# ofsouzap/DistributedMandelbrot

Measured on AMD Instinct MI355X. Metric: G pixel-iterations/s on 4096^2 tile, max_iter=1000 fp64, higher is better.
Workload: dtype f64

## Files before the change

distributedmandelbrot_amd/_lib.py:

```python
from __future__ import annotations

import ctypes as C
import importlib.util
import os
import sys

HERE = os.path.dirname(os.path.abspath(__file__))
SO_PATH = os.path.join(HERE, "libmbk_hip.so")

MBK_OK, MBK_ERR_INVALID, MBK_ERR_NO_DEVICE, MBK_ERR_HIP, MBK_ERR_NOMEM, MBK_ERR_NET = range(6)
MBK_WANT_COUNTS = 0x1
MBK_WANT_BYTES = 0x2
MBK_KERNEL_DEFAULT = 0x000
MBK_KERNEL_SIMPLE = 0x100
MBK_KERNEL_ASM = 0x200
MBK_KERNEL_REFILL = 0x300
MBK_KERNEL_GROUP = 0x400
MBK_KERNEL_SCAN = 0x500
KERNELS = {"default": MBK_KERNEL_DEFAULT, "simple": MBK_KERNEL_SIMPLE, "asm": MBK_KERNEL_ASM,
           "refill": MBK_KERNEL_REFILL, "group": MBK_KERNEL_GROUP, "scan": MBK_KERNEL_SCAN}
OPTIONS = {name: i for i, name in enumerate(
    ["order", "waves_per_wg", "group_steps", "exact_steps", "probe_steps", "scan_waves", "scan_xcd_map", "scan_col_period", "heavy_share",
     "rf_livemin", "rf_patience", "rf_batch", "rf_waves", "cycle_detect", "probe_mid", "prepass_overlap", "exact_long", "scan_inline", "wave_limit", "units_min_light", "xcd_balance", "m_late", "h_settled", "classify_wg", "scan_strip", "cycle_window", "spill_first", "spill_lanes", "spill_min_mrd", "spill_min_blocks", "spill_cyc_shift"])}
MBK_PRECISION_F32 = 0x1000
MBK_LAZY_UNIFORM = 0x2000
MBK_DEEP_BLA = 0x8000
MBK_DEEP_XBLA = 0x10000
PRECISIONS = {"f64": 0, "f32": MBK_PRECISION_F32}
MBK_SLOTS = 4
MBK_WORKER_DEPTH = 3
MBK_INFO_SCAN_WG_PER_CU = 100
MBK_INFO_XCD_SHARE = 110
MBK_INFO_SPILL = 130
MBK_CODEC_RAW = 0x00
MBK_CODEC_RLE = 0x01
MBK_CHUNK_DEFINITION = 4096
MBK_CHUNK_BYTES = 4096 * 4096
MBK_ABI_VERSION = 5
# ... 137 lines not shown
    "mbk_distance_value_host": (C.c_double, [C.c_double, C.c_double, C.c_int32]),
    "mbk_datachunk_submit": (C.c_int, [C.c_void_p, C.c_int, C.c_uint32, C.c_uint32, C.c_uint32, C.c_uint32,
                                       C.c_void_p, C.c_void_p]),
    "mbk_datachunk_submit_ex": (C.c_int, [C.c_void_p, C.c_int, C.c_uint32, C.c_uint32, C.c_uint32, C.c_uint32,
                                          C.c_void_p, C.c_void_p, C.c_uint32]),
    "mbk_view_submit": (C.c_int, [C.c_void_p, C.c_int, C.POINTER(mbk_view), C.c_uint32, C.c_uint32,
                                  C.c_void_p, C.c_void_p]),
    "mbk_wait": (C.c_int, [C.c_void_p, C.c_int, C.POINTER(mbk_stats)]),
    "mbk_serialize_last": (C.c_int, [C.c_void_p, C.c_void_p, C.c_uint64, C.POINTER(C.c_uint64),
                                     C.POINTER(C.c_uint32)]),
    "mbk_set_option": (C.c_int, [C.c_void_p, C.c_int, C.c_uint32]),
    "mbk_get_option": (C.c_int, [C.c_void_p, C.c_int, C.POINTER(C.c_uint32)]),
    "mbk_quantise_counts": (C.c_int, [C.c_void_p, C.c_void_p, C.c_uint64, C.c_uint32, C.c_void_p]),
    "mbk_units_plan": (C.c_int, [C.c_uint32, C.c_uint32, C.c_uint32, C.c_void_p, C.c_void_p]),
    "mbk_units_lookup": (C.c_int, [C.c_void_p, C.c_uint32, C.c_void_p, C.c_void_p]),
    "mbk_reduce_counts": (C.c_int, [C.c_void_p, C.c_void_p, C.c_uint64, C.c_uint32, C.c_void_p,
                                    C.POINTER(mbk_stats)]),
    "mbk_worker_run": (C.c_int, [C.c_void_p, C.c_char_p, C.c_uint16, C.c_uint64, C.c_uint32,
                                 C.POINTER(mbk_worker_report)]),
    "mbk_net_set_option": (C.c_int, [C.c_int, C.c_uint32]),
    "mbk_net_get_option": (C.c_int, [C.c_int, C.POINTER(C.c_uint32)]),
    "mbk_feeder_run": (C.c_int, [C.POINTER(mbk_feeder_ops), C.c_char_p, C.c_uint16, C.c_uint64, C.c_uint32,
                                 C.POINTER(mbk_worker_report)]),
    "mbk_deep_orbit_create": (C.c_int, [C.c_char_p, C.c_char_p, C.c_uint32, C.c_uint32, C.POINTER(C.c_void_p)]),
    "mbk_deep_orbit_destroy": (None, [C.c_void_p]),
    "mbk_deep_orbit_info": (C.c_int, [C.c_void_p, C.POINTER(C.c_uint32), C.POINTER(C.c_uint32), C.POINTER(C.c_uint32),
                                      C.POINTER(C.c_uint32)]),
    "mbk_deep_orbit_read": (C.c_int, [C.c_void_p, C.c_void_p, C.c_void_p, C.c_uint64]),
    "mbk_deep_view_launch": (C.c_int, [C.c_void_p, C.c_void_p, C.POINTER(mbk_deep_view), C.c_uint32, C.c_uint32,
                                       C.c_void_p, C.c_void_p, C.c_void_p, C.c_void_p]),
# ... 193 lines not shown
```

distributedmandelbrot_amd/csrc/mbk_api.hip:

```cpp
#include "../../include/mbk.h"

#include <hip/hip_runtime.h>

#include <cmath>
#include <cstdio>
#include <cstdlib>
#include <algorithm>
#include <cstring>
#include <new>
#include <string>
#include <vector>

#include "mbk_kernels.h"
#include "mbk_refill.h"
#include "mbk_persist.h"
#include "mbk_scan.h"
#include "mbk_units.h"
#include "mbk_spill.h"
#include "mbk_feeder.h"
#include "mbk_deep_orbit.h"
#include "mbk_deep.h"
#include "mbk_deep_bla.h"
#include "mbk_deep_wide.h"
#include "mbk_deep_wide_bla.h"
// ... 1042 lines not shown
    if (wb && mrd == 0) return fail(ctx, MBK_ERR_INVALID, "mrd == 0 has no quantised form (division by zero)");

    TileArgs a;
    std::memset(&a, 0, sizeof(a));
    fill_window(a, v);
    a.out_pitch = v->ncols;
    a.out_col0 = 0;
    a.out_row0 = 0;
    a.mrd = (int32_t)mrd;
    a.quant_wide = (mrd >= (1u << 23)) ? 1u : 0u;
    a.quant_rcp = mrd ? 1.0 / (double)mrd : 0.0;
    a.perm_mul = 1u;
    a.exact_steps = ctx->opt[MBK_OPT_EXACT_STEPS];
    a.exact_steps_long = std::min(ctx->opt[MBK_OPT_EXACT_STEPS], ctx->opt[MBK_OPT_EXACT_LONG]);
    a.cyc_window = ctx->opt[MBK_OPT_CYCLE_WINDOW];
    a.order = nullptr;
    a.counts = wc ? d_counts : nullptr;
    a.bytes = wb ? d_bytes : nullptr;
    a.smooth = d_smooth;

    const uint32_t kernel = flags & MBK_KERNEL_MASK;
    if (d_smooth && (f32 || kernel == MBK_KERNEL_SIMPLE || kernel == MBK_KERNEL_REFILL))
        return fail(ctx, MBK_ERR_INVALID, "smooth colouring is implemented by the fp64 scan / asm / group kernels only");
    if (f32 && (kernel == MBK_KERNEL_SIMPLE || kernel == MBK_KERNEL_REFILL))
        return fail(ctx, MBK_ERR_INVALID, "MBK_PRECISION_F32 is implemented by the scan / asm / group kernels only");
    switch (kernel) {
        case MBK_KERNEL_DEFAULT:
        case MBK_KERNEL_SCAN: {
            if (kernel == MBK_KERNEL_DEFAULT && (uint64_t)((a.ncols + 7u) / 8u) * ((a.nrows + 7u) / 8u) < 16384u)
                return launch_blocks(ctx, a, MBK_KERNEL_GROUP, safe, f32, stream);
// ... 415 lines not shown
    hipError_t e = hipGetDeviceCount(&n);
    if (e != hipSuccess || n <= 0)
        return fail(nullptr, MBK_ERR_NO_DEVICE,
                    std::string("no HIP device visible (") + hipGetErrorString(e) +
                        "); libmbk_hip has no CPU fallback");
    if (device < 0 || device >= n) return fail(nullptr, MBK_ERR_NO_DEVICE, "device index out of range");
    mbk_ctx *ctx = new (std::nothrow) mbk_ctx();
    if (!ctx) return fail(nullptr, MBK_ERR_NOMEM, "out of host memory");
    ctx->device = device;
    static const uint32_t kDefaults[MBK_OPT_COUNT_] = {
         3u,  1u,  16u,  8u,  32u,
         8u,  1u,  4u,  655u,
         48u,  256u,  1u,  8u,  1u,
         65537u,  1u,  0u,  1u,  0u,
         32768u,  0u,  8u,  6u,  1024u,
         1u,  32u,  256u,  16u,  2048u,  19u,  5u};
    std::memcpy(ctx->opt, kDefaults, sizeof(kDefaults));
#define MBK_CREATE_HIP(call)                                                        \
    do {                                                                            \
        hipError_t e2_ = (call);                                                    \
        if (e2_ != hipSuccess) {                                                    \
            fail(nullptr, MBK_ERR_HIP, std::string(#call) + ": " + hipGetErrorString(e2_)); \
            mbk_destroy(ctx);                                                       \
            return MBK_ERR_HIP;                                                     \
        }                                                                           \
    } while (0)
    MBK_CREATE_HIP(hipSetDevice(device));
    MBK_CREATE_HIP(hipGetDeviceProperties(&ctx->prop, device));
    if (std::strncmp(ctx->prop.gcnArchName, "gfx950", 6) != 0) {
        fail(nullptr, MBK_ERR_NO_DEVICE,
             std::string("device is ") + ctx->prop.gcnArchName + ", this library is built for gfx950 only");
// ... 604 lines not shown
        case MBK_OPT_CLASSIFY_WG: ok = value >= 64u && value <= 1024u && value % 64u == 0u; break;
        case MBK_OPT_SCAN_STRIP: ok = value <= 1u; break;
        case MBK_OPT_CYCLE_WINDOW: ok = value <= 65536u; break;
        case MBK_OPT_EXACT_LONG: ok = value <= 4096u; break;
        case MBK_OPT_SCAN_INLINE: ok = value <= 1u; break;
        case MBK_OPT_WAVE_LIMIT: ok = value <= 7u; break;
        case MBK_OPT_UNITS_MIN_LIGHT: ok = value <= 65536u; break;
        case MBK_OPT_XCD_BALANCE: ok = value <= 2u; break;
        case MBK_OPT_M_LATE: ok = value <= 65536u; break;
        case MBK_OPT_H_SETTLED: ok = value <= 30u; break;
        case MBK_OPT_SPILL_FIRST: ok = value <= 65536u && value % 32u == 0u; break;
        case MBK_OPT_SPILL_LANES: ok = value >= 1u && value <= 32u; break;
        case MBK_OPT_SPILL_MIN_MRD: ok = true; break;
        case MBK_OPT_SPILL_MIN_BLOCKS: ok = value <= 31u; break;
        case MBK_OPT_SPILL_CYC_SHIFT: ok = value <= 31u; break;
        default: return fail(ctx, MBK_ERR_INVALID, "unknown MBK_OPT_* selector");
    }
    if (!ok) return fail(ctx, MBK_ERR_INVALID, "option value out of range");
    ctx->opt[option] = value;
    return MBK_OK;
}

int mbk_get_option(mbk_ctx *ctx, int option, uint32_t *value)
{
    if (!ctx || !value) return fail(ctx, MBK_ERR_INVALID, "NULL argument");
    if (option >= MBK_INFO_SCAN_WG_PER_CU && option < MBK_INFO_SCAN_WG_PER_CU + 4) {
        const int k = option - MBK_INFO_SCAN_WG_PER_CU;
        *value = (uint32_t)ctx->scan_occ[k >> 1][k & 1];
        return MBK_OK;
    }
// ... 30 lines not shown
    double c = 0.0;
    for (uint32_t x = 0; x < 8u; ++x) {
        c += f[x];
        cum[x] = x == 7u ? (1u << 24) : (uint32_t)std::lround(std::min(1.0, std::max(0.0, c)) * (double)(1u << 24));
    }
}

int mbk_units_plan(uint32_t n_h, uint32_t n_v, uint32_t n_m, const double *fractions, uint32_t *plan)
{
    if (!fractions || !plan) return MBK_ERR_INVALID;
    if ((uint64_t)n_h + n_v + n_m > 0x7fffffffull) return MBK_ERR_INVALID;
    uint32_t cum[8];
    shares_from_fractions(fractions, cum);
    mbk::units_plan(n_h, n_v, n_m, cum, 0u, plan, 0u, 0u);
    return MBK_OK;
}

int mbk_units_lookup(const uint32_t *plan, uint32_t id, uint32_t *list, uint32_t *index)
{
    if (!plan || !list || !index) return MBK_ERR_INVALID;
    const uint32_t x = id & 7u;
    bool is_h = false;
    uint32_t i = 0;
    *list = 0u;
    *index = 0u;
    if (id >= plan[2] || !mbk::units_lookup(id, plan[3], plan[4], plan[8u + x], plan[16u + x], plan[24u + x], plan[32u + x], is_h, i))
        return MBK_OK;
    *list = is_h ? 1u : (i < plan[1] ? 2u : 3u);
    *index = is_h ? i : (i < plan[1] ? i : i - plan[1]);
    return MBK_OK;
// ... 2275 lines not shown
```

distributedmandelbrot_amd/csrc/mbk_kernels.h:

```cpp
#pragma once

#include <hip/hip_runtime.h>
#include <stdint.h>

namespace mbk {

struct Axis {
    double start;
    double step;
    double last;
    double delta;
    double div;
    uint32_t n;
    uint32_t step_is_zero;
};

struct ReduceSlot;

constexpr uint32_t kSpillLevels = 12;

struct TileArgs {
    Axis re, im;
    uint32_t col0, row0, ncols, nrows;
    uint32_t blocks_x;
// ... 12 lines not shown
    uint32_t unit_stride;
    uint32_t stamp_tag;
    const uint32_t *plan;
    unsigned long long *stamps;
    int32_t *counts;
    uint8_t *bytes;
    double *smooth;
    ReduceSlot *stats;
    uint32_t cyc_window;
    uint32_t spill_first;
    uint32_t spill_lanes;
    uint32_t spill_win_shift;
    void *spill_z;
    uint32_t *spill_meta;
    uint32_t *spill_cnt;
};

__device__ __forceinline__ double axis_value(const Axis &a, uint32_t k)
{
    double y;
    if (a.step_is_zero) {
        double q = (double)k / a.div;
        y = q * a.delta;
    } else {
        y = (double)k * a.step;
    }
    double v = y + a.start;
    return (k + 1u == a.n) ? a.last : v;
}

// ... 78 lines not shown
#undef MBK_CYC_MOV
#define MBK_T float
#define MBK_F "f32"
#define MBK_CI_FROM_T64 "v_add_f64 %[t64], %[t64], %[start]\nv_cvt_f32_f64 %[ci], %[t64]\n"
#define MBK_CR_FROM_T64 "v_add_f64 %[t64], %[t64], %[start]\nv_cvt_f32_f64 %[cr], %[t64]\n"
#define MBK_CYC_BITS "u32"
#define MBK_CYC_MOV "b32"
#include "mbk_loops.inc"
#undef MBK_T
#undef MBK_F
#undef MBK_CI_FROM_T64
#undef MBK_CR_FROM_T64
#undef MBK_CYC_BITS
#undef MBK_CYC_MOV


template <typename T, bool kFmaDouble, int kGroup, bool kCycle = false>
__device__ __forceinline__ int32_t block_pixel(const TileArgs &p, uint32_t ucol, uint32_t urow, uint32_t lx, uint32_t ly,
                                               bool long_groups, bool interior = false)
{
    const uint32_t lc = ucol + lx, lr = urow + ly;
    T cr, ci;
    bool ring_test = kGroup != 0 && kFmaDouble;
    if (interior) {
        cr = (T)((double)(p.col0 + lc) * p.re.step + p.re.start);
        ci = (T)((double)(p.row0 + lr) * p.im.step + p.im.start);
        ring_test = ring_test && p.ring_possible != 0u;
    } else {
        if (lc >= p.ncols || lr >= p.nrows) return -1;
        cr = (T)axis_value(p.re, p.col0 + lc);
        ci = (T)axis_value(p.im, p.row0 + lr);
    }
    int32_t count;
    T m = 0;
    if (kGroup != 0 && kFmaDouble) {
        bool risky = false;
        if (ring_test) {
            const T c2 = cr * cr + ci * ci;
            const T margin = sizeof(T) == 8 ? (T)1e-9 : (T)1e-3;
            risky = __ballot(__builtin_fabs((double)(c2 - (T)4)) < (double)margin) != 0ull;
        }
        if (risky) {
            count = escape_count_asm<true>(cr, ci, p.mrd, &m);
        } else if (kGroup == 32) {
            count = long_groups ? escape_count_group<32, false>(cr, ci, p.mrd, &m, p.exact_steps_long)
                                : escape_count_group<8, false>(cr, ci, p.mrd, &m, p.exact_steps);
        } else if (kGroup == 16) {
            count = long_groups ? escape_count_group<16, kCycle>(cr, ci, p.mrd, &m, p.exact_steps_long, p.cyc_window)
                                : escape_count_group<8, kCycle>(cr, ci, p.mrd, &m, p.exact_steps, p.cyc_window);
        } else {
            count = escape_count_group<kGroup == 8 ? 8 : 4, kCycle>(cr, ci, p.mrd, &m, p.exact_steps, p.cyc_window);
        }
    } else {
        count = escape_count_asm<kFmaDouble>(cr, ci, p.mrd, &m);
    }
    const size_t ubase = (size_t)(urow + p.out_row0) * p.out_pitch + ucol + p.out_col0;
    const uint32_t loff = ly * p.out_pitch + lx;
    if (p.counts) (p.counts + ubase)[loff] = count;
    if (p.bytes) (p.bytes + ubase)[loff] = quantise(count, p);
    if (p.smooth) (p.smooth + ubase)[loff] = smooth_value(count, (double)m);
    return count;
}

template <typename T> struct SpillPair;
template <> struct SpillPair<double> { using type = double2; };
template <> struct SpillPair<float> { using type = float2; };
constexpr int32_t kSpilled = -2;

template <typename T, int kGroup, bool kCycle>
__device__ __forceinline__ void block_pixel_spill(const TileArgs &p, uint32_t ucol, uint32_t urow, uint32_t lx, uint32_t ly,
                                                  bool long_groups, uint32_t block_index)
{
// ... 90 lines not shown
            e = (j >= n_heavy && j < n_heavy + n_mid) ? p.order[p.ngrid + 3u + (j - n_heavy)] : p.order[j];
        } else {
            e = p.order[j];
            n_heavy = p.order[p.ngrid];
        }
        by = e >> 16;
        bx = e & 0xffffu;
    } else {
        const uint32_t blk = (uint32_t)(((uint64_t)blockIdx.x * p.perm_mul) % gridDim.x);
        by = blk / p.blocks_x;
        bx = blk - by * p.blocks_x;
    }
    const uint32_t wcol = bx * (blockDim.x >> 6) + wave;
    const bool long_groups = kGroup >= 16 && (!p.order || (blockIdx.x >= heavy_lo && blockIdx.x < heavy_lo + n_heavy));
    const bool interior = wcol < p.fast_bx_end && by < p.fast_by_end;
    if (kSpill && kFmaDouble && kGroup >= 8 && interior)
        block_pixel_spill<T, kGroup, kCycle>(p, wcol * 8u, by * 8u, lane & 7u, lane >> 3, long_groups, by * p.blocks_x + wcol);
    else
    block_pixel<T, kFmaDouble, kGroup, kCycle>(p, wcol * 8u, by * 8u, lane & 7u, lane >> 3, long_groups, interior);
}

__global__ __launch_bounds__(1024) void classify_blocks_kernel(TileArgs p, uint32_t nregions,
                                                                uint32_t region_w, int32_t probe_steps, int32_t mid_min,
                                                                uint32_t *order, uint32_t *counters)
{
    __shared__ uint32_t s_cnt[3][16], s_base[3];
    const uint32_t r = blockIdx.x * blockDim.x + threadIdx.x;
    const uint32_t lane = threadIdx.x & 63u, wave = threadIdx.x >> 6;
    const bool valid = r < nregions;
    uint32_t cls = 1u;
    uint32_t packed = 0;
    if (valid) {
        const uint32_t by = r / p.blocks_x, bx = r - by * p.blocks_x;
        packed = (by << 16) | bx;
// ... 255 lines not shown
```

distributedmandelbrot_amd/csrc/mbk_units.h:

```cpp
#pragma once

#include "mbk_refill.h"

namespace mbk {

__host__ __device__ inline size_t units_settled_base(size_t n) { return 2u * n + 64u; }
__host__ __device__ inline size_t units_list_words(size_t n) { return 3u * n + 64u; }

struct XcdShares { uint32_t cum[8]; };
__host__ __device__ inline void units_plan(uint32_t n_h, uint32_t n_v, uint32_t n_m, const uint32_t *cum, uint32_t stamps, uint32_t *plan,
                                           uint32_t n_ml, uint32_t n_hs);

__device__ __forceinline__ int32_t probe_settling(double cr, double ci, int32_t cap, double *delta)
{
    double zr = cr, zi = ci;
    int32_t n = 1;
    for (; n < cap - 9; ++n) {
        const double t = zr * zr - zi * zi;
        zi = __builtin_fma(2.0, zr * zi, ci);
        zr = t + cr;
        if (zr * zr + zi * zi >= 4.0) { *delta = 1e300; return n; }
    }
    double hr[9], hi[9];
#pragma unroll
// ... 193 lines not shown
        load_shares(args.plan, x, n_m, total, hmin, lmin, stamps, n_ml, hs0, h_x, l_x, hbase_x, lbase_x);
        if (stamps && u < p.unit_stride) {
            const uint32_t j0 = u >> 3, slots = total >> 3;
            if (j0 == 0u) leave_stamp(x);
            if (j0 < slots && j0 + kStampTail >= slots) leave_stamp(8u + x * kStampTail + (j0 + kStampTail - slots));
        }
        if (u >= total) break;
        bool is_h;
        uint32_t i;
        if (!units_lookup(u, hmin, lmin, h_x, l_x, hbase_x, lbase_x, is_h, i)) break;
        if (is_h || i < n_m) {
            const bool late = is_h && i < n_ml;
            const uint32_t e = scalar_load_u32(p.order, is_h ? (late ? 2u * n + 2u - i : (i < hs0 ? i - n_ml : (uint32_t)units_settled_base(n) + (i - hs0)))
                                                              : n + 3u + i);
            const uint32_t by = e >> 16, bx = e & 0xffffu;
            const int32_t c = block_pixel<T, true, kGroup, kCycle>(p, bx * 8u, by * 8u, lx, ly, kGroup >= 16 && is_h && !late,
                                                                   bx < p.fast_bx_end && by < p.fast_by_end);
            if (kStats && c >= 0) heavy += c > 0 ? (unsigned long long)(uint32_t)c : (1ull << 47) + never_cap;
        } else {
            const uint32_t v = scalar_load_u32(p.order, n - 1u - (i - n_m));
            const uint32_t by = v >> 16, bx0 = ((v >> 8) & 0xffu) << 3, mask = v & 0xffu;
            const T ci = (T)((double)(p.row0 + by * 8u + ly) * p.im.step + p.im.start);
            const T b0 = ci * ci;
            const size_t elem0 = (size_t)(by * 8u + p.out_row0) * p.out_pitch + bx0 * 8u + p.out_col0;
            int32_t *cb = reinterpret_cast<int32_t *>(uniform_u64(reinterpret_cast<unsigned long long>(kCounts ? p.counts + elem0 : nullptr)));
            uint8_t *bb = reinterpret_cast<uint8_t *>(uniform_u64(reinterpret_cast<unsigned long long>(kBytes ? p.bytes + elem0 : nullptr)));
            const uint32_t col = p.col0 + bx0 * 8u + lx, off = (ly * p.out_pitch + lx) * oscale;
            uint32_t k = 0;
            int32_t cnt;
            while (escape_light_row<kCounts, kBytes, kStats>(ci, b0, col, p.re.step, p.re.start, cnt, cb, bb, off, 8u * oscale, qtab, mask, k, &acc) != 0u) {
                const int32_t c = block_pixel<T, true, kGroup, kCycle>(p, (bx0 + k) * 8u, by * 8u, lx, ly, false, true);
                if (kStats && c >= 0) heavy += c > 0 ? (unsigned long long)(uint32_t)c : (1ull << 47) + never_cap;
// ... 16 lines not shown
```

distributedmandelbrot_amd/device.py:

```python
from __future__ import annotations

import ctypes as C
import math
from dataclasses import dataclass
from decimal import Decimal
from fractions import Fraction
from typing import Optional, Tuple, Union

import numpy as np

from . import _lib as L


class MbkError(RuntimeError):
    def __init__(self, status: int, message: str):
        super().__init__(f"libmbk_hip status {status}: {message}")
        self.status = status


def _error_text(lib, ctx=None) -> str:
    return (lib.mbk_last_error(ctx) or b"").decode()


def _check(lib, st: int, ctx=None) -> None:
# ... 414 lines not shown
        self._check(self._lib.mbk_device_pci_bus_id(self._h, buf, 32))
        return buf.value.decode()

    def pinned_empty(self, shape, dtype) -> np.ndarray:
        dtype = np.dtype(dtype)
        n = int(np.prod(shape)) * dtype.itemsize
        p = C.c_void_p()
        self._check(self._lib.mbk_host_alloc(self._h, max(n, 1), C.byref(p)))
        self._pinned.append(p)
        buf = (C.c_uint8 * max(n, 1)).from_address(p.value)
        return np.frombuffer(buf, dtype=dtype, count=int(np.prod(shape))).reshape(shape)

    def set_option(self, name: str, value: int) -> None:
        self._check(self._lib.mbk_set_option(self._h, L.OPTIONS[name], int(value)))

    def get_option(self, name: str) -> int:
        v = C.c_uint32(0)
        self._check(self._lib.mbk_get_option(self._h, L.OPTIONS[name], C.byref(v)))
        return int(v.value)

    def scan_occupancy(self) -> dict:
        out = {}
        for k, name in enumerate(["f64_scan", "f64_heavy", "f32_scan", "f32_heavy"]):
            v = C.c_uint32(0)
            self._check(self._lib.mbk_get_option(self._h, L.MBK_INFO_SCAN_WG_PER_CU + k, C.byref(v)))
            out[name] = int(v.value)
        return out

    def xcd_shares(self) -> dict:
        vals = []
# ... 502 lines not shown
```

include/mbk.h:

```cpp
#ifndef MBK_H
#define MBK_H

#include <stdint.h>

#ifdef __cplusplus
extern "C" {
#endif

#define MBK_ABI_VERSION 5

#define MBK_CHUNK_DEFINITION 4096u
#define MBK_CHUNK_BYTES (4096u * 4096u)

enum mbk_status {
    MBK_OK = 0,
    MBK_ERR_INVALID = 1,
    MBK_ERR_NO_DEVICE = 2,
    MBK_ERR_HIP = 3,
    MBK_ERR_NOMEM = 4,
    MBK_ERR_NET = 5
};

#define MBK_WANT_COUNTS 0x1u
#define MBK_WANT_BYTES 0x2u
// ... 356 lines not shown
    MBK_OPT_EXACT_LONG,
    MBK_OPT_SCAN_INLINE,
    MBK_OPT_WAVE_LIMIT,
    MBK_OPT_UNITS_MIN_LIGHT,
    MBK_OPT_XCD_BALANCE,
    MBK_OPT_M_LATE,
    MBK_OPT_H_SETTLED,
    MBK_OPT_CLASSIFY_WG,
    MBK_OPT_SCAN_STRIP,
    MBK_OPT_CYCLE_WINDOW,
    MBK_OPT_SPILL_FIRST,
    MBK_OPT_SPILL_LANES,
    MBK_OPT_SPILL_MIN_MRD,
    MBK_OPT_SPILL_MIN_BLOCKS,
    MBK_OPT_SPILL_CYC_SHIFT,
    MBK_OPT_COUNT_
};
#define MBK_INFO_SCAN_WG_PER_CU 100
#define MBK_INFO_XCD_SHARE 110
#define MBK_INFO_SPILL 130
int mbk_set_option(mbk_ctx *ctx, int option, uint32_t value);
int mbk_get_option(mbk_ctx *ctx, int option, uint32_t *value);

int mbk_units_plan(uint32_t n_h, uint32_t n_v, uint32_t n_m, const double *fractions, uint32_t *plan);
int mbk_units_lookup(const uint32_t *plan, uint32_t id, uint32_t *list, uint32_t *index);

int mbk_quantise_counts(mbk_ctx *ctx, const int32_t *h_counts, uint64_t n, uint32_t mrd, uint8_t *h_bytes);

int mbk_reduce_counts(mbk_ctx *ctx, const int32_t *d_counts, uint64_t n, uint32_t mrd,
                      void *hip_stream, mbk_stats *stats);

typedef struct mbk_worker_report {
    uint64_t leased;
    uint64_t accepted;
    uint64_t rejected;
    uint64_t resets;
    uint64_t uniform_tiles;
    uint64_t pixel_iterations;
    double kernel_ms_sum;
    double seconds;
// ... 35 lines not shown
```

profiles/microbench/units_classes.hip:

```cpp
#include <hip/hip_runtime.h>
#include <cmath>
#include <cstdio>
#include <cstdlib>
#include <cstring>
#include <string>
#include <vector>
#include "../../distributedmandelbrot_amd/csrc/mbk_units.h"

#define CHECK(x) do { hipError_t e_ = (x); if (e_ != hipSuccess) { printf("HIP error %s at line %d\n", hipGetErrorString(e_), __LINE__); exit(1); } } while (0)

template <bool kCycle, int kClass>
__global__ __launch_bounds__(64) __attribute__((amdgpu_waves_per_eu(8, 8))) void class_units_kernel(mbk::TileArgs args, uint32_t qtab, uint32_t u0)
{
    mbk::TileArgs p = args;
    p.smooth = nullptr; p.stats = nullptr; p.quant_wide = 0u; p.re.step_is_zero = p.im.step_is_zero = 0u; p.bytes = nullptr;
    const uint32_t lane = threadIdx.x, lx = lane & 7u, ly = lane >> 3;
    const uint32_t n = p.ngrid;
    const uint32_t n_h = mbk::uniform_u32(p.order[n]), n_v = mbk::uniform_u32(p.order[n + 1u]), n_m = mbk::uniform_u32(p.order[n + 2u]);
    const uint32_t n_ml = mbk::uniform_u32(p.order[2u * n + 3u]), n_hs = mbk::uniform_u32(p.order[2u * n + 4u]);
    const uint32_t u = blockIdx.x + u0;
    if (u < n_ml + n_h + n_hs + n_m) {
        const bool late = u < n_ml, is_hu = !late && u < n_ml + n_h, is_hs = !late && !is_hu && u < n_ml + n_h + n_hs;
        const uint32_t e = mbk::uniform_u32(late ? p.order[2u * n + 2u - u] : is_hu ? p.order[u - n_ml]
                                            : is_hs ? p.order[mbk::units_settled_base(n) + (u - n_ml - n_h)] : p.order[n + 3u + (u - n_ml - n_h - n_hs)]);
        const uint32_t by = e >> 16, bx = e & 0xffffu;
        mbk::block_pixel<double, true, 16, kCycle>(p, bx * 8u, by * 8u, lx, ly, is_hu || is_hs, bx < p.fast_bx_end && by < p.fast_by_end);
    } else if (u < n_ml + n_h + n_hs + n_m + n_v) {
        const uint32_t v = mbk::uniform_u32(p.order[n - 1u - (u - n_ml - n_h - n_hs - n_m)]);
        const uint32_t by = v >> 16, bx0 = ((v >> 8) & 0xffu) << 3, mask = v & 0xffu;
        const double ci = (double)(p.row0 + by * 8u + ly) * p.im.step + p.im.start, b0 = ci * ci;
        const size_t elem0 = (size_t)(by * 8u + p.out_row0) * p.out_pitch + bx0 * 8u + p.out_col0;
        int32_t *cb = reinterpret_cast<int32_t *>(mbk::uniform_u64(reinterpret_cast<unsigned long long>(p.counts + elem0)));
        const uint32_t col = p.col0 + bx0 * 8u + lx, off = (ly * p.out_pitch + lx) * 4u;
        uint32_t k = 0;
        int32_t cnt;
        while (mbk::escape_light_row<true, false>(ci, b0, col, p.re.step, p.re.start, cnt, cb, nullptr, off, 32u, qtab, mask, k) != 0u) {
            mbk::block_pixel<double, true, 16, kCycle>(p, (bx0 + k) * 8u, by * 8u, lx, ly, false, true);
            if (++k >= 8u) break;
        }
    }
}

template <bool kCycle>
static void launch_class(int cls, uint32_t grid, const mbk::TileArgs &a, uint32_t u0)
{
    if (grid == 0) return;
    switch (cls) {
        case 0: class_units_kernel<kCycle, 0><<<grid, 64>>>(a, 0u, u0); break;
        case 1: class_units_kernel<kCycle, 1><<<grid, 64>>>(a, 0u, u0); break;
        case 2: class_units_kernel<kCycle, 2><<<grid, 64>>>(a, 0u, u0); break;
        case 3: class_units_kernel<kCycle, 3><<<grid, 64>>>(a, 0u, u0); break;
        case 4: class_units_kernel<kCycle, 4><<<grid, 64>>>(a, 0u, u0); break;
        default: class_units_kernel<kCycle, 5><<<grid, 64>>>(a, 0u, u0); break;
    }
}

int main(int argc, char **argv)
{
    const std::string wl = argc > 1 ? argv[1] : "cfg2";
    const bool cyc = argc > 2 && atoi(argv[2]) != 0;
    const int m_late = argc > 3 ? atoi(argv[3]) : 8;
    const int h_settled = cyc ? (argc > 4 ? atoi(argv[4]) : 6) : 0;
    const double settle_thr = h_settled ? pow(10.0, -(double)h_settled) : 0.0;
    const uint32_t W = 4096, H = 4096, mrd = 1000;
    mbk::TileArgs a; memset(&a, 0, sizeof(a));
    auto mk = [](double start, double range, uint32_t n) { mbk::Axis x; memset(&x, 0, sizeof(x)); x.start = start; x.n = n;
        volatile double stop = start + range, delta = stop - start, div = n - 1, step = delta / div;
        x.last = stop; x.delta = delta; x.div = div; x.step = step; x.step_is_zero = 0; return x; };
    if (wl == "chunk_l1") { a.re = mk(-2.0, 4.0, W); a.im = mk(-2.0, 4.0, H); }
    else { a.re = mk(-2.0, 3.0, W); a.im = mk(-1.5, 3.0, H); }
    a.ncols = W; a.nrows = H; a.out_pitch = W; a.mrd = mrd; a.quant_rcp = 1.0 / mrd;
    a.exact_steps = 8; a.exact_steps_long = 0; a.ring_possible = 1; a.cyc_window = 32;
    a.blocks_x = W / 8;
    a.fast_bx_end = W / 8 - 1; a.fast_by_end = H / 8 - 1;
    a.perm_mul = 1;
    const uint32_t nblocks = a.blocks_x * (H / 8);
    CHECK(hipMalloc(&a.counts, (size_t)W * H * 4));
    uint32_t *ord; CHECK(hipMalloc(&ord, mbk::units_list_words(nblocks) * 4));
    a.order = ord; a.ngrid = nblocks; a.unit_stride = nblocks;
    CHECK(hipMemset(ord + nblocks, 0, 12));
    CHECK(hipMemset(ord + 2 * (size_t)nblocks + 3, 0, 8));
    mbk::classify_units_kernel<<<(nblocks + 1023) / 1024, 1024>>>(a, nblocks, 32, ord, ord + nblocks, m_late, settle_thr, ord + 2 * (size_t)nblocks + 3, nullptr, mbk::XcdShares(), 0u);
    std::vector<uint32_t> lst(mbk::units_list_words(nblocks));
    CHECK(hipMemcpy(lst.data(), ord, lst.size() * 4, hipMemcpyDeviceToHost));
    const uint32_t n = nblocks, n_h = lst[n], n_v = lst[n + 1], n_m = lst[n + 2], n_ml = lst[2 * (size_t)n + 3], n_hs = lst[2 * (size_t)n + 4];
    const uint32_t size[6] = {n_ml + n_h + n_hs + n_m + n_v, n_ml, n_h, n_hs, n_m, n_v};
    const uint32_t first[6] = {0, 0, n_ml, n_ml + n_h, n_ml + n_h + n_hs, n_ml + n_h + n_hs + n_m};
// ... 29 lines not shown
    unsigned long long iters[6] = {0, 0, 0, 0, 0, 0}, wsteps[6] = {0, 0, 0, 0, 0, 0};
    for (uint32_t u = 0; u < size[0]; ++u) {
        int c;
        if (u < first[2]) c = 1; else if (u < first[3]) c = 2; else if (u < first[4]) c = 3; else if (u < first[5]) c = 4; else c = 5;
        if (c < 5) {
            const uint32_t e = c == 1 ? lst[2 * (size_t)n + 2 - u] : c == 2 ? lst[u - n_ml] : c == 3 ? lst[mbk::units_settled_base(n) + (u - n_ml - n_h)]
                                                                                              : lst[n + 3 + (u - n_ml - n_h - n_hs)];
            block_work(e & 0xffffu, e >> 16, iters[c], wsteps[c]);
        } else {
            const uint32_t v = lst[n - 1 - (u - first[5])];
            const uint32_t by = v >> 16, bx0 = ((v >> 8) & 0xffu) << 3, mask = v & 0xffu;
            for (uint32_t k = 0; k < 8; ++k) if (mask >> k & 1u) block_work(bx0 + k, by, iters[c], wsteps[c]);
        }
    }
    for (int c = 1; c < 6; ++c) { iters[0] += iters[c]; wsteps[0] += wsteps[c]; }
    printf("%s, cycle test %d, m_late %d, h_settled %d: strict work per class from the counts (a pixel's iterations = count, or mrd - 1 = %u for a never-escaping one; "
           "wave-steps = the block's longest pixel, what a lock-step wave runs WITHOUT the cycle test)\n", wl.c_str(), (int)cyc, m_late, h_settled, mrd - 1);
    printf("%-10s %9s %16s %14s %10s %12s\n", "class", "entries", "pixel-iterations", "wave-steps", "activity", "ms alone");
    for (int c = 0; c < 6; ++c)
        printf("%-10s %9u %16llu %14llu %10.4f %12.4f\n", names[c], size[c], iters[c], wsteps[c], wsteps[c] ? (double)iters[c] / 64.0 / (double)wsteps[c] : 0.0, ms[c]);
    return 0;
}
```

Baseline: 5228.

## Add attracting-cycle trap certificate to end interior pixels early in heavy blocks

For each pixel in the main cardioid or period-2 bulb region, it computes a certified trap disk around the attracting fixed point or 2-cycle. The heavy-block iteration loop then runs in doubling segments and marks a pixel as never-escaping once z falls inside the disk. The aim is to skip the remaining iterations for interior pixels that the cycle detector catches late or never. In exchange it adds per-pixel certificate setup (complex sqrt, float maths), extra wave ballots at segment boundaries and more register pressure. It is enabled by default through a new option.

```diff
diff --git a/distributedmandelbrot_amd/_lib.py b/distributedmandelbrot_amd/_lib.py
--- a/distributedmandelbrot_amd/_lib.py
+++ b/distributedmandelbrot_amd/_lib.py
@@ -21,7 +21,7 @@
            "refill": MBK_KERNEL_REFILL, "group": MBK_KERNEL_GROUP, "scan": MBK_KERNEL_SCAN}
 OPTIONS = {name: i for i, name in enumerate(
     ["order", "waves_per_wg", "group_steps", "exact_steps", "probe_steps", "scan_waves", "scan_xcd_map", "scan_col_period", "heavy_share",
-     "rf_livemin", "rf_patience", "rf_batch", "rf_waves", "cycle_detect", "probe_mid", "prepass_overlap", "exact_long", "scan_inline", "wave_limit", "units_min_light", "xcd_balance", "m_late", "h_settled", "classify_wg", "scan_strip", "cycle_window", "spill_first", "spill_lanes", "spill_min_mrd", "spill_min_blocks", "spill_cyc_shift"])}
+     "rf_livemin", "rf_patience", "rf_batch", "rf_waves", "cycle_detect", "probe_mid", "prepass_overlap", "exact_long", "scan_inline", "wave_limit", "units_min_light", "xcd_balance", "m_late", "h_settled", "classify_wg", "scan_strip", "cycle_window", "spill_first", "spill_lanes", "spill_min_mrd", "spill_min_blocks", "spill_cyc_shift", "trap"])}
 MBK_PRECISION_F32 = 0x1000
 MBK_LAZY_UNIFORM = 0x2000
 MBK_DEEP_BLA = 0x8000
@@ -189,6 +189,8 @@
     "mbk_quantise_counts": (C.c_int, [C.c_void_p, C.c_void_p, C.c_uint64, C.c_uint32, C.c_void_p]),
     "mbk_units_plan": (C.c_int, [C.c_uint32, C.c_uint32, C.c_uint32, C.c_void_p, C.c_void_p]),
     "mbk_units_lookup": (C.c_int, [C.c_void_p, C.c_uint32, C.c_void_p, C.c_void_p]),
+    "mbk_trap_certificate": (C.c_int, [C.c_double, C.c_double, C.c_void_p]),
+    "mbk_trap_inside": (C.c_int, [C.c_double, C.c_double, C.c_double, C.c_double]),
     "mbk_reduce_counts": (C.c_int, [C.c_void_p, C.c_void_p, C.c_uint64, C.c_uint32, C.c_void_p,
                                     C.POINTER(mbk_stats)]),
     "mbk_worker_run": (C.c_int, [C.c_void_p, C.c_char_p, C.c_uint16, C.c_uint64, C.c_uint32,
diff --git a/distributedmandelbrot_amd/csrc/mbk_api.hip b/distributedmandelbrot_amd/csrc/mbk_api.hip
--- a/distributedmandelbrot_amd/csrc/mbk_api.hip
+++ b/distributedmandelbrot_amd/csrc/mbk_api.hip
@@ -1080,6 +1080,7 @@
     a.exact_steps = ctx->opt[MBK_OPT_EXACT_STEPS];
     a.exact_steps_long = std::min(ctx->opt[MBK_OPT_EXACT_STEPS], ctx->opt[MBK_OPT_EXACT_LONG]);
     a.cyc_window = ctx->opt[MBK_OPT_CYCLE_WINDOW];
+    a.trap = ctx->opt[MBK_OPT_TRAP];
     a.order = nullptr;
     a.counts = wc ? d_counts : nullptr;
     a.bytes = wb ? d_bytes : nullptr;
@@ -1525,7 +1526,7 @@
          48u,  256u,  1u,  8u,  1u,
          65537u,  1u,  0u,  1u,  0u,
          32768u,  0u,  8u,  6u,  1024u,
-         1u,  32u,  256u,  16u,  2048u,  19u,  5u};
+         1u,  32u,  256u,  16u,  2048u,  19u,  5u,  1u};
     std::memcpy(ctx->opt, kDefaults, sizeof(kDefaults));
 #define MBK_CREATE_HIP(call)                                                        \
     do {                                                                            \
@@ -2160,6 +2161,7 @@
         case MBK_OPT_SPILL_MIN_MRD: ok = true; break;
         case MBK_OPT_SPILL_MIN_BLOCKS: ok = value <= 31u; break;
         case MBK_OPT_SPILL_CYC_SHIFT: ok = value <= 31u; break;
+        case MBK_OPT_TRAP: ok = value <= 1u; break;
         default: return fail(ctx, MBK_ERR_INVALID, "unknown MBK_OPT_* selector");
     }
     if (!ok) return fail(ctx, MBK_ERR_INVALID, "option value out of range");
@@ -2220,6 +2222,28 @@
     shares_from_fractions(fractions, cum);
     mbk::units_plan(n_h, n_v, n_m, cum, 0u, plan, 0u, 0u);
     return MBK_OK;
+}
+
+int mbk_trap_certificate(double cr, double ci, double *out)
+{
+    if (!out) return MBK_ERR_INVALID;
+    const mbk::TrapProof t = mbk::trap_prove(cr, ci);
+    out[0] = (double)t.period;
+    out[1] = t.a1r;
+    out[2] = t.a1i;
+    out[3] = t.a2r;
+    out[4] = t.a2i;
+    out[5] = t.r1;
+    out[6] = t.r2;
+    out[7] = (double)mbk::trap_r1sq(t.cert);
+    out[8] = (double)mbk::trap_r2sq(t.cert);
+    return MBK_OK;
+}
+
+int mbk_trap_inside(double cr, double ci, double zr, double zi)
+{
+    const mbk::TrapCert c = mbk::trap_prove(cr, ci).cert;
+    return c.rsq != 0u && mbk::trap_inside(c, zr, zi) ? 1 : 0;
 }
 
 int mbk_units_lookup(const uint32_t *plan, uint32_t id, uint32_t *list, uint32_t *index)
diff --git a/distributedmandelbrot_amd/csrc/mbk_kernels.h b/distributedmandelbrot_amd/csrc/mbk_kernels.h
--- a/distributedmandelbrot_amd/csrc/mbk_kernels.h
+++ b/distributedmandelbrot_amd/csrc/mbk_kernels.h
@@ -2,6 +2,9 @@
 
 #include <hip/hip_runtime.h>
 #include <stdint.h>
+#include <type_traits>
+
+#include "mbk_trap.h"
 
 namespace mbk {
 
@@ -50,6 +53,7 @@
     void *spill_z;
     uint32_t *spill_meta;
     uint32_t *spill_cnt;
+    uint32_t trap;
 };
 
 __device__ __forceinline__ double axis_value(const Axis &a, uint32_t k)
@@ -158,10 +162,45 @@
 #undef MBK_CYC_BITS
 #undef MBK_CYC_MOV
 
-
-template <typename T, bool kFmaDouble, int kGroup, bool kCycle = false>
+template <int kGroup>
+__device__ __forceinline__ int32_t escape_count_trap(double cr, double ci, int32_t mrd, double *m_out, uint32_t exact_steps, uint32_t cyc_wcap)
+{
+    static_assert(kGroup == 8 || kGroup == 16, "8- or 16-step groups");
+    TrapCert tc = trap_prove(cr, ci).cert;
+    double zr = cr, zi = ci;
+    double a = zr * zr, b = zi * zi, m = 0;
+    int32_t cnt = 0;
+    const uint32_t total = mrd > 1 ? (uint32_t)mrd - 1u : 0u;
+    const uint32_t first = total < exact_steps ? total : exact_steps;
+    escape_steps_asm<true>(cr, ci, zr, zi, a, b, m, cnt, 0u, first);
+    double szr = zr, szi = zi;
+    uint32_t cyc_tc = 0u, cyc_win = 1u;
+    uint32_t n = first, k = 0u;
+    while (n < total) {
+        if (__ballot(cnt == 0) == 0ull) break;
+        uint32_t stop = total;
+        if (__ballot(cnt == 0 && tc.rsq != 0u) != 0ull) {
+            const uint32_t sh = k < 4u ? 0u : (k - 2u) >> 1, seg = 16u << (sh < 26u ? sh : 26u);
+            if (total - n > seg) stop = n + seg;
+        }
+        if (cnt == 0) escape_steps_carry<kGroup>(cr, ci, zr, zi, a, b, m, cnt, n, stop, cyc_wcap, szr, szi, cyc_tc, cyc_win);
+        cyc_tc = (uint32_t)__builtin_amdgcn_readfirstlane((int)cyc_tc);
+        cyc_win = (uint32_t)__builtin_amdgcn_readfirstlane((int)cyc_win);
+        n = stop;
+        ++k;
+        if (n >= total) break;
+        asm volatile("" : "+v"(tc.ar), "+v"(tc.ai), "+v"(tc.rsq));
+        if (cnt == 0 && tc.rsq != 0u && trap_inside(tc, zr, zi)) cnt = -1;
+    }
+    escape_fixup(cr, ci, zr, zi, a, b, m, cnt);
+    if (m_out) *m_out = m;
+    return cnt < 0 ? 0 : cnt;
+}
+
+
+template <typename T, bool kFmaDouble, int kGroup, bool kCycle = false, bool kTrapForm = false>
 __device__ __forceinline__ int32_t block_pixel(const TileArgs &p, uint32_t ucol, uint32_t urow, uint32_t lx, uint32_t ly,
-                                               bool long_groups, bool interior = false)
+                                               bool long_groups, bool interior = false, bool trap = false)
 {
     const uint32_t lc = ucol + lx, lr = urow + ly;
     T cr, ci;
@@ -184,8 +223,14 @@
             const T margin = sizeof(T) == 8 ? (T)1e-9 : (T)1e-3;
             risky = __ballot(__builtin_fabs((double)(c2 - (T)4)) < (double)margin) != 0ull;
         }
+        constexpr bool kTrap = kTrapForm && kCycle && std::is_same<T, double>::value && (kGroup == 8 || kGroup == 16);
         if (risky) {
             count = escape_count_asm<true>(cr, ci, p.mrd, &m);
+        } else if (kTrap && trap) {
+            if constexpr (kTrap) {
+                count = (kGroup == 16 && long_groups) ? escape_count_trap<16>(cr, ci, p.mrd, &m, p.exact_steps_long, p.cyc_window)
+                                                      : escape_count_trap<8>(cr, ci, p.mrd, &m, p.exact_steps, p.cyc_window);
+            }
         } else if (kGroup == 32) {
             count = long_groups ? escape_count_group<32, false>(cr, ci, p.mrd, &m, p.exact_steps_long)
                                 : escape_count_group<8, false>(cr, ci, p.mrd, &m, p.exact_steps);
@@ -199,7 +244,9 @@
         count = escape_count_asm<kFmaDouble>(cr, ci, p.mrd, &m);
     }
     const size_t ubase = (size_t)(urow + p.out_row0) * p.out_pitch + ucol + p.out_col0;
-    const uint32_t loff = ly * p.out_pitch + lx;
+    uint32_t sx = lx, sy = ly;
+    if (kTrapForm) asm volatile("" : "+v"(sx), "+v"(sy));
+    const uint32_t loff = sy * p.out_pitch + sx;
     if (p.counts) (p.counts + ubase)[loff] = count;
     if (p.bytes) (p.bytes + ubase)[loff] = quantise(count, p);
     if (p.smooth) (p.smooth + ubase)[loff] = smooth_value(count, (double)m);
@@ -320,10 +367,11 @@
     const uint32_t wcol = bx * (blockDim.x >> 6) + wave;
     const bool long_groups = kGroup >= 16 && (!p.order || (blockIdx.x >= heavy_lo && blockIdx.x < heavy_lo + n_heavy));
     const bool interior = wcol < p.fast_bx_end && by < p.fast_by_end;
+    const bool trap = kCycle && !kSpill && p.trap != 0u && (!p.order || (blockIdx.x >= heavy_lo && blockIdx.x < heavy_lo + n_heavy));
     if (kSpill && kFmaDouble && kGroup >= 8 && interior)
         block_pixel_spill<T, kGroup, kCycle>(p, wcol * 8u, by * 8u, lane & 7u, lane >> 3, long_groups, by * p.blocks_x + wcol);
     else
-    block_pixel<T, kFmaDouble, kGroup, kCycle>(p, wcol * 8u, by * 8u, lane & 7u, lane >> 3, long_groups, interior);
+    block_pixel<T, kFmaDouble, kGroup, kCycle, kCycle && !kSpill && std::is_same<T, double>::value>(p, wcol * 8u, by * 8u, lane & 7u, lane >> 3, long_groups, interior, trap);
 }
 
 __global__ __launch_bounds__(1024) void classify_blocks_kernel(TileArgs p, uint32_t nregions,
diff --git a/distributedmandelbrot_amd/csrc/mbk_trap.h b/distributedmandelbrot_amd/csrc/mbk_trap.h
--- /dev/null
+++ b/distributedmandelbrot_amd/csrc/mbk_trap.h
@@ -0,0 +1,147 @@
+#pragma once
+
+#include <hip/hip_runtime.h>
+#include <stdint.h>
+
+namespace mbk {
+
+constexpr double kTrapDelta = 0x1p-40;
+constexpr double kTrapMinGap = 0x1p-8;
+constexpr double kTrapMaxAbs = 1.5;
+constexpr double kTrapShrink = 1.0 - 0x1p-20;
+
+struct TrapCert {
+    float ar, ai;
+    uint32_t rsq;
+};
+__host__ __device__ __forceinline__ float trap_bits_float(uint32_t u)
+{
+    float f;
+    __builtin_memcpy(&f, &u, sizeof(u));
+    return f;
+}
+__host__ __device__ __forceinline__ float trap_r1sq(const TrapCert &c) { return trap_bits_float(c.rsq & 0xffff0000u); }
+__host__ __device__ __forceinline__ float trap_r2sq(const TrapCert &c) { return trap_bits_float(c.rsq << 16); }
+struct TrapProof {
+    int period;
+    double a1r, a1i, a2r, a2i, r1, r2;
+    TrapCert cert;
+};
+
+__host__ __device__ __forceinline__ float trap_sqrtf(float x)
+{
+#if defined(__HIP_DEVICE_COMPILE__)
+    return __builtin_amdgcn_sqrtf(x);
+#else
+    return __builtin_sqrtf(x);
+#endif
+}
+__host__ __device__ __forceinline__ float trap_rcpf(float x)
+{
+#if defined(__HIP_DEVICE_COMPILE__)
+    return __builtin_amdgcn_rcpf(x);
+#else
+    return 1.0f / x;
+#endif
+}
+
+__host__ __device__ __forceinline__ double trap_abs_up(double x, double y)
+{
+    return (double)trap_sqrtf((float)(x * x + y * y)) * (1.0 + 0x1p-20) + 0x1p-40;
+}
+__host__ __device__ __forceinline__ double trap_abs1(double x, double y)
+{
+    return __builtin_fabs(x) + __builtin_fabs(y);
+}
+__host__ __device__ __forceinline__ uint32_t trap_half_down(double x)
+{
+    const float f = (float)x;
+    uint32_t u;
+    __builtin_memcpy(&u, &f, sizeof(u));
+    u -= (double)f > x ? 1u : 0u;
+    return u >> 16;
+}
+__host__ __device__ __forceinline__ void trap_csqrtf(double qr, double qi, float &wr, float &wi)
+{
+    const float fr = (float)qr, fi = (float)qi;
+    const float h = trap_sqrtf(fr * fr + fi * fi);
+    const float s = trap_sqrtf(0.5f * (h + __builtin_fabsf(fr)));
+    const float o = 0.5f * __builtin_fabsf(fi) * trap_rcpf(s);
+    wr = fr >= 0.0f ? s : o;
+    wi = __builtin_copysignf(fr >= 0.0f ? o : s, fi);
+}
+
+__host__ __device__ __forceinline__ bool trap_period1(double cr, double ci, TrapProof &t)
+{
+    float wr, wi;
+    trap_csqrtf(0.25 - cr, -ci, wr, wi);
+    const float arf = 0.5f - wr, aif = -wi;
+    const double ar = (double)arf, ai = (double)aif;
+    const double la = trap_abs_up(ar, ai);
+    const double gap = 1.0 - 2.0 * la;
+    const double e = trap_abs1(ar * ar - ai * ai + cr - ar, 2.0 * ar * ai + ci - ai);
+    const double r = 0.5 * gap;
+    if (!(gap >= kTrapMinGap && r * (gap - r) >= e + kTrapDelta && la + r <= kTrapMaxAbs)) return false;
+    t.period = 1;
+    t.a1r = t.a2r = ar;
+    t.a1i = t.a2i = ai;
+    t.r1 = t.r2 = r;
+    t.cert.ar = arf;
+    t.cert.ai = aif;
+    t.cert.rsq = trap_half_down(r * r * kTrapShrink) << 16;
+    return true;
+}
+
+__host__ __device__ __forceinline__ bool trap_period2(double cr, double ci, TrapProof &t)
+{
+    float wr, wi;
+    trap_csqrtf(-3.0 - 4.0 * cr, -4.0 * ci, wr, wi);
+    const float a1rf = 0.5f * wr - 0.5f, a1if = 0.5f * wi;
+    const double a1r = (double)a1rf, a1i = (double)a1if;
+    const double a2r = -1.0 - a1r, a2i = -a1i;
+    const double la1 = trap_abs_up(a1r, a1i), la2 = trap_abs_up(a2r, a2i);
+    const double gap = 1.0 - 4.0 * la1 * la2;
+    if (!(gap >= kTrapMinGap)) return false;
+    const double e1 = trap_abs1(a1r * a1r - a1i * a1i + cr - a2r, 2.0 * a1r * a1i + ci - a2i);
+    const double e2 = trap_abs1(a2r * a2r - a2i * a2i + cr - a1r, 2.0 * a2r * a2i + ci - a1i);
+    for (double r1 = 0.25 * gap; r1 >= 0x1p-6 * gap; r1 *= 0.5) {
+        const double r2 = e1 + 2.0 * la1 * r1 + r1 * r1 + kTrapDelta;
+        const double back = e2 + 2.0 * la2 * r2 + r2 * r2 + kTrapDelta;
+        if (back <= r1 && la1 + r1 <= kTrapMaxAbs && la2 + r2 <= kTrapMaxAbs) {
+            t.period = 2;
+            t.a1r = a1r;
+            t.a1i = a1i;
+            t.a2r = a2r;
+            t.a2i = a2i;
+            t.r1 = r1;
+            t.r2 = r2;
+            t.cert.ar = a1rf;
+            t.cert.ai = a1if;
+            t.cert.rsq = (trap_half_down(r1 * r1 * kTrapShrink) << 16) | trap_half_down(r2 * r2 * kTrapShrink);
+            return true;
+        }
+    }
+    return false;
+}
+
+__host__ __device__ __forceinline__ TrapProof trap_prove(double cr, double ci)
+{
+    TrapProof t;
+    t.period = 0;
+    t.a1r = t.a1i = t.a2r = t.a2i = t.r1 = t.r2 = 0.0;
+    t.cert.ar = t.cert.ai = 0.0f;
+    t.cert.rsq = 0u;
+    if (!(__builtin_fabs(cr + 0.4375) <= 0.8125 && __builtin_fabs(ci) <= 0.65625)) return t;
+    if (!trap_period1(cr, ci, t)) trap_period2(cr, ci, t);
+    return t;
+}
+
+__host__ __device__ __forceinline__ bool trap_inside(const TrapCert &c, double zr, double zi)
+{
+    const double ar = (double)c.ar, ai = (double)c.ai;
+    const double d1r = zr - ar, d1i = zi - ai;
+    const double d2r = zr - (-1.0 - ar), d2i = zi + ai;
+    return d1r * d1r + d1i * d1i < (double)trap_r1sq(c) || d2r * d2r + d2i * d2i < (double)trap_r2sq(c);
+}
+
+}
diff --git a/distributedmandelbrot_amd/csrc/mbk_units.h b/distributedmandelbrot_amd/csrc/mbk_units.h
--- a/distributedmandelbrot_amd/csrc/mbk_units.h
+++ b/distributedmandelbrot_amd/csrc/mbk_units.h
@@ -231,8 +231,8 @@
             const uint32_t e = scalar_load_u32(p.order, is_h ? (late ? 2u * n + 2u - i : (i < hs0 ? i - n_ml : (uint32_t)units_settled_base(n) + (i - hs0)))
                                                               : n + 3u + i);
             const uint32_t by = e >> 16, bx = e & 0xffffu;
-            const int32_t c = block_pixel<T, true, kGroup, kCycle>(p, bx * 8u, by * 8u, lx, ly, kGroup >= 16 && is_h && !late,
-                                                                   bx < p.fast_bx_end && by < p.fast_by_end);
+            const int32_t c = block_pixel<T, true, kGroup, kCycle, kCycle && std::is_same<T, double>::value>(p, bx * 8u, by * 8u, lx, ly, kGroup >= 16 && is_h && !late,
+                                                                   bx < p.fast_bx_end && by < p.fast_by_end, kCycle && p.trap != 0u && is_h && !late);
             if (kStats && c >= 0) heavy += c > 0 ? (unsigned long long)(uint32_t)c : (1ull << 47) + never_cap;
         } else {
             const uint32_t v = scalar_load_u32(p.order, n - 1u - (i - n_m));
diff --git a/distributedmandelbrot_amd/device.py b/distributedmandelbrot_amd/device.py
--- a/distributedmandelbrot_amd/device.py
+++ b/distributedmandelbrot_amd/device.py
@@ -452,6 +452,14 @@
     def set_option(self, name: str, value: int) -> None:
         self._check(self._lib.mbk_set_option(self._h, L.OPTIONS[name], int(value)))
 
+    @staticmethod
+    def trap_certificate(cr: float, ci: float) -> dict:
+        out = (C.c_double * 10)()
+        if L.load().mbk_trap_certificate(float(cr), float(ci), out) != 0:
+            raise ValueError("mbk_trap_certificate failed")
+        return {"period": int(out[0]), "a1": complex(out[1], out[2]), "a2": complex(out[3], out[4]), "r1": out[5], "r2": out[6],
+                "r1sq": out[7], "r2sq": out[8]}
+
     def get_option(self, name: str) -> int:
         v = C.c_uint32(0)
         self._check(self._lib.mbk_get_option(self._h, L.OPTIONS[name], C.byref(v)))
diff --git a/include/mbk.h b/include/mbk.h
--- a/include/mbk.h
+++ b/include/mbk.h
@@ -394,6 +394,7 @@
     MBK_OPT_SPILL_MIN_MRD,
     MBK_OPT_SPILL_MIN_BLOCKS,
     MBK_OPT_SPILL_CYC_SHIFT,
+    MBK_OPT_TRAP,
     MBK_OPT_COUNT_
 };
 #define MBK_INFO_SCAN_WG_PER_CU 100
@@ -404,6 +405,9 @@
 
 int mbk_units_plan(uint32_t n_h, uint32_t n_v, uint32_t n_m, const double *fractions, uint32_t *plan);
 int mbk_units_lookup(const uint32_t *plan, uint32_t id, uint32_t *list, uint32_t *index);
+
+int mbk_trap_certificate(double cr, double ci, double *out);
+int mbk_trap_inside(double cr, double ci, double zr, double zi);
 
 int mbk_quantise_counts(mbk_ctx *ctx, const int32_t *h_counts, uint64_t n, uint32_t mrd, uint8_t *h_bytes);
 
diff --git a/profiles/microbench/units_classes.hip b/profiles/microbench/units_classes.hip
--- a/profiles/microbench/units_classes.hip
+++ b/profiles/microbench/units_classes.hip
@@ -24,7 +24,8 @@
         const uint32_t e = mbk::uniform_u32(late ? p.order[2u * n + 2u - u] : is_hu ? p.order[u - n_ml]
                                             : is_hs ? p.order[mbk::units_settled_base(n) + (u - n_ml - n_h)] : p.order[n + 3u + (u - n_ml - n_h - n_hs)]);
         const uint32_t by = e >> 16, bx = e & 0xffffu;
-        mbk::block_pixel<double, true, 16, kCycle>(p, bx * 8u, by * 8u, lx, ly, is_hu || is_hs, bx < p.fast_bx_end && by < p.fast_by_end);
+        mbk::block_pixel<double, true, 16, kCycle, kCycle>(p, bx * 8u, by * 8u, lx, ly, is_hu || is_hs, bx < p.fast_bx_end && by < p.fast_by_end,
+                                                           kCycle && p.trap != 0u && (is_hu || is_hs));
     } else if (u < n_ml + n_h + n_hs + n_m + n_v) {
         const uint32_t v = mbk::uniform_u32(p.order[n - 1u - (u - n_ml - n_h - n_hs - n_m)]);
         const uint32_t by = v >> 16, bx0 = ((v >> 8) & 0xffu) << 3, mask = v & 0xffu;
@@ -35,7 +36,7 @@
         uint32_t k = 0;
         int32_t cnt;
         while (mbk::escape_light_row<true, false>(ci, b0, col, p.re.step, p.re.start, cnt, cb, nullptr, off, 32u, qtab, mask, k) != 0u) {
-            mbk::block_pixel<double, true, 16, kCycle>(p, (bx0 + k) * 8u, by * 8u, lx, ly, false, true);
+            mbk::block_pixel<double, true, 16, kCycle, kCycle>(p, (bx0 + k) * 8u, by * 8u, lx, ly, false, true);
             if (++k >= 8u) break;
         }
     }
@@ -61,6 +62,7 @@
     const bool cyc = argc > 2 && atoi(argv[2]) != 0;
     const int m_late = argc > 3 ? atoi(argv[3]) : 8;
     const int h_settled = cyc ? (argc > 4 ? atoi(argv[4]) : 6) : 0;
+    const uint32_t trap = cyc && argc > 5 ? (uint32_t)atoi(argv[5]) : 0u;
     const double settle_thr = h_settled ? pow(10.0, -(double)h_settled) : 0.0;
     const uint32_t W = 4096, H = 4096, mrd = 1000;
     mbk::TileArgs a; memset(&a, 0, sizeof(a));
@@ -70,7 +72,7 @@
     if (wl == "chunk_l1") { a.re = mk(-2.0, 4.0, W); a.im = mk(-2.0, 4.0, H); }
     else { a.re = mk(-2.0, 3.0, W); a.im = mk(-1.5, 3.0, H); }
     a.ncols = W; a.nrows = H; a.out_pitch = W; a.mrd = mrd; a.quant_rcp = 1.0 / mrd;
-    a.exact_steps = 8; a.exact_steps_long = 0; a.ring_possible = 1; a.cyc_window = 32;
+    a.exact_steps = 8; a.exact_steps_long = 0; a.ring_possible = 1; a.cyc_window = 32; a.trap = trap;
     a.blocks_x = W / 8;
     a.fast_bx_end = W / 8 - 1; a.fast_by_end = H / 8 - 1;
     a.perm_mul = 1;
@@ -130,8 +132,8 @@
         }
     }
     for (int c = 1; c < 6; ++c) { iters[0] += iters[c]; wsteps[0] += wsteps[c]; }
-    printf("%s, cycle test %d, m_late %d, h_settled %d: strict work per class from the counts (a pixel's iterations = count, or mrd - 1 = %u for a never-escaping one; "
-           "wave-steps = the block's longest pixel, what a lock-step wave runs WITHOUT the cycle test)\n", wl.c_str(), (int)cyc, m_late, h_settled, mrd - 1);
+    printf("%s, cycle test %d, m_late %d, h_settled %d, trap %u: strict work per class from the counts (a pixel's iterations = count, or mrd - 1 = %u for a never-escaping one; "
+           "wave-steps = the block's longest pixel, what a lock-step wave runs WITHOUT the cycle test)\n", wl.c_str(), (int)cyc, m_late, h_settled, trap, mrd - 1);
     printf("%-10s %9s %16s %14s %10s %12s\n", "class", "entries", "pixel-iterations", "wave-steps", "activity", "ms alone");
     for (int c = 0; c < 6; ++c)
         printf("%-10s %9u %16llu %14llu %10.4f %12.4f\n", names[c], size[c], iters[c], wsteps[c], wsteps[c] ? (double)iters[c] / 64.0 / (double)wsteps[c] : 0.0, ms[c]);
```

After: 5227, median of 2. About the same (-0.0%).
